# CuzImSlymi/Apertis-LLM

Hardware: AMD Instinct MI355X
Metric: train tokens/sec/node (seq=4096) (higher is better)
Workload: dtype bf16

## Files before the change

### apertis_llm_amd/csrc/moe_routing.hip

```cpp
#include "row_common.h"

namespace {

template <int EC>
__global__ void gate_topk_fwd_k(const float *__restrict__ logits, float *__restrict__ gates,
                                int32_t *__restrict__ idx, float *__restrict__ w, int64_t S, int E_rt,
                                int K) {
  const int64_t s = (int64_t)blockIdx.x * blockDim.x + threadIdx.x;
  if (s >= S) return;
  const int E = EC > 0 ? EC : E_rt;
  gate_topk_row<EC>(logits + s * E, gates + s * E, idx + s * K, w + s * K, E_rt, K);
}

template <int EC>
__global__ void gate_topk_bwd_k(const float *__restrict__ gates, const int32_t *__restrict__ idx,
                                const float *__restrict__ dw, const float *__restrict__ dgates,
                                float *__restrict__ dlogits, int64_t S, int E_rt, int K) {
  const int64_t s = (int64_t)blockIdx.x * blockDim.x + threadIdx.x;
  if (s >= S) return;
  constexpr int CAP = EC > 0 ? EC : MAXE;
  const int E = EC > 0 ? EC : E_rt;
  float g[CAP], dg[CAP];
#pragma unroll
  for (int i = 0; i < CAP; ++i)
    if (i < E) { g[i] = gates[s * E + i]; dg[i] = dgates ? dgates[s * E + i] : 0.f; }
  if (dw) {
    float psum = 0.f, dot = 0.f;
    for (int k = 0; k < K; ++k) {
      int e = idx[s * K + k];
      float pe = 0.f;
#pragma unroll
      for (int i = 0; i < CAP; ++i)
        if (i == e) pe = g[i];
      psum += pe;
      dot += dw[s * K + k] * pe;
    }
    const float den = psum + 1e-6f;
    const float corr = dot / (den * den);
    for (int k = 0; k < K; ++k) {
      int e = idx[s * K + k];
      float dp = dw[s * K + k] / den - corr;
#pragma unroll
      for (int i = 0; i < CAP; ++i)
        if (i == e) dg[i] += dp;
    }
  }
  float inner = 0.f;
#pragma unroll
  for (int i = 0; i < CAP; ++i)
    if (i < E) inner += dg[i] * g[i];
#pragma unroll
  for (int i = 0; i < CAP; ++i)
    if (i < E) dlogits[s * E + i] = g[i] * (dg[i] - inner);
}

constexpr int PLAN_HIST_BLOCKS = 512;
struct PlanWs {
  int32_t *total, *keep, *mode, *quota, *seg_start, *bpart;
  uint32_t *thr, *smask;
  int32_t *ghist;
  int32_t *done;
  int32_t *cnt_g, *cnt_t;
  int P, NCH;
};

PlanWs carve_ws(void *ws, int64_t S, int64_t E, int64_t K) {
  PlanWs w;
  w.P = (int)(E * K);
  w.NCH = (int)ceil_div64(S, 64);
  int32_t *p = (int32_t *)ws;
  w.total = p; p += w.P;
  w.keep = p; p += w.P;
  w.mode = p; p += w.P;
  w.quota = p; p += w.P;
  w.seg_start = p; p += w.P;
  w.thr = (uint32_t *)p; p += w.P;
  w.smask = (uint32_t *)p; p += w.P;
  w.ghist = p; p += (int64_t)w.P * 256;
  w.done = p; p += 4;
  w.cnt_g = p; p += (int64_t)w.P * w.NCH;
  w.cnt_t = p; p += (int64_t)w.P * w.NCH;
  w.bpart = p;
  return w;
}

__global__ void __launch_bounds__(256)
plan_hist_k(const int32_t *__restrict__ idx, int32_t *__restrict__ bpart, int64_t SK, int E, int K) {
  __shared__ int32_t h[MAXE * MAXK];
  const int P = E * K, lane = threadIdx.x & 63;
  for (int i = threadIdx.x; i < P; i += blockDim.x) h[i] = 0;
  __syncthreads();
  for (int64_t a0 = (int64_t)blockIdx.x * blockDim.x; a0 < SK; a0 += (int64_t)gridDim.x * blockDim.x) {
    const int64_t a = a0 + threadIdx.x;
    int slot = -1;
    if (a < SK) {
      const int e = idx[a];
      if (e >= 0 && e < E) slot = e * K + (int)(a % K);
    }
    unsigned long long todo = __ballot(slot >= 0);
    while (todo) {
      const int leader = __ffsll((long long)todo) - 1;
      const int s0 = __shfl(slot, leader);
      const unsigned long long m = __ballot(slot == s0);
      if (lane == leader) atomicAdd(&h[s0], __popcll(m));
      todo &= ~m;
    }
  }
  __syncthreads();
  for (int i = threadIdx.x; i < P; i += blockDim.x) bpart[(int64_t)blockIdx.x * P + i] = h[i];
}

__global__ void plan_capacity_k(PlanWs w, const uint8_t *__restrict__ active, int64_t capacity,
                                int32_t *__restrict__ offsets, int E, int K, int nhist) {
  __shared__ int32_t s_sum[256];
  {
    const int P = E * K;
    const int g = P < 256 ? 256 / P : 1;
    for (int p0 = 0; p0 < P; p0 += 256 / g) {
      const int p = p0 + (int)threadIdx.x / g, sub = (int)threadIdx.x % g;
      int t = 0;
      if (p < P && (int)threadIdx.x / g < 256 / g)
        for (int b = sub; b < nhist; b += g) t += w.bpart[(int64_t)b * P + p];
      s_sum[threadIdx.x] = t;
      __syncthreads();
      if (p < P && sub == 0 && (int)threadIdx.x / g < 256 / g) {
        int tt = 0;
        for (int q = 0; q < g; ++q) tt += s_sum[threadIdx.x + q];
        w.total[p] = tt;
      }
      __syncthreads();
    }
  }
  const int e = threadIdx.x;
  if (e < E) {
    int64_t load = 0;
    const bool on = active ? active[e] != 0 : true;
    for (int k = 0; k < K; ++k) {
      const int p = e * K + k;
      const int tot = w.total[p];
      int64_t keep = tot;
      if (!on) keep = 0;
      else if (capacity > 0) {
        int64_t rem = capacity - load;
        keep = rem <= 0 ? 0 : (tot < rem ? tot : rem);
      }
      w.keep[p] = (int)keep;
      w.mode[p] = keep == 0 ? 0 : (keep == tot ? 1 : 2);
      w.quota[p] = (int)keep;
      w.thr[p] = 0;
      w.smask[p] = 0;
      load += keep;
    }
  }
  __syncthreads();
  if (threadIdx.x == 0) {
    int run = 0;
    for (int ee = 0; ee < E; ++ee) {
      offsets[ee] = run;
      for (int k = 0; k < K; ++k) {
        w.seg_start[ee * K + k] = run;
        run += w.keep[ee * K + k];
      }
    }
    offsets[E] = run;
  }
}

__global__ void __launch_bounds__(1024)
plan_select_k(PlanWs w, const int32_t *__restrict__ idx, const float *__restrict__ wk, int64_t S, int K) {
  const int p = blockIdx.x;
  if (w.mode[p] != 2) return;
  const int e = p / K, k = p - e * K;
  __shared__ int32_t hist[256];
  __shared__ uint32_t s_prefix, s_mask;
  __shared__ int32_t s_need;
  if (threadIdx.x == 0) { s_prefix = 0; s_mask = 0; s_need = w.keep[p]; }
  for (int shift = 24; shift >= 0; shift -= 8) {
    for (int i = threadIdx.x; i < 256; i += blockDim.x) hist[i] = 0;
    __syncthreads();
    const uint32_t prefix = s_prefix, mask = s_mask;
    for (int64_t s0 = threadIdx.x; s0 < S; s0 += (int64_t)blockDim.x * 8) {
      int32_t ei[8];
      uint32_t bi[8];
#pragma unroll
      for (int u = 0; u < 8; ++u) {
        const int64_t s = s0 + (int64_t)u * blockDim.x;
        ei[u] = s < S ? idx[s * K + k] : -1;
        bi[u] = s < S ? __float_as_uint(wk[s * K + k]) : 0u;
      }
#pragma unroll
      for (int u = 0; u < 8; ++u)
        if (ei[u] == e && (bi[u] & mask) == prefix) atomicAdd(&hist[(bi[u] >> shift) & 255], 1);
    }
    __syncthreads();
    if (threadIdx.x == 0) {
      int need = s_need, cum = 0;
      for (int b = 255; b >= 0; --b) {
        if (cum + hist[b] >= need) {
          s_need = need - cum;
          s_prefix = prefix | ((uint32_t)b << shift);
          s_mask = mask | (255u << shift);
          break;
        }
        cum += hist[b];
      }
    }
    __syncthreads();
  }
  if (threadIdx.x == 0) { w.thr[p] = s_prefix; w.quota[p] = s_need; }
}

__device__ __forceinline__ void plan_sel_pick(const PlanWs &w, int p, int lane, int shift) {
  if (w.mode[p] != 2) return;
  int32_t *h = w.ghist + p * 256;
  int c[4];
#pragma unroll
  for (int j = 0; j < 4; ++j) c[j] = __hip_atomic_load(h + 255 - 4 * lane - j, __ATOMIC_RELAXED, __HIP_MEMORY_SCOPE_AGENT);
  const int mine = (c[0] + c[1]) + (c[2] + c[3]);
  int incl = mine;
#pragma unroll
  for (int off = 1; off < 64; off <<= 1) {
    const int v = __shfl_up(incl, off);
    if (lane >= off) incl += v;
  }
  const int need = w.quota[p];
  const int before = incl - mine;
  if (before < need && incl >= need) {
    int cum = before, b = 0;
#pragma unroll
    for (int j = 0; j < 4; ++j) {
      if (cum < need && cum + c[j] >= need) { b = 255 - 4 * lane - j; break; }
      cum += c[j];
    }
    w.quota[p] = need - cum;
    w.thr[p] = w.thr[p] | ((uint32_t)b << shift);
    w.smask[p] = w.smask[p] | (255u << shift);
  }
#pragma unroll
  for (int j = 0; j < 4; ++j) h[255 - 4 * lane - j] = 0;
}

__global__ void __launch_bounds__(256)
plan_sel_hist_k(PlanWs w, const int32_t *__restrict__ idx, const float *__restrict__ wk, int64_t S, int E, int K, int shift, int digit) {
  extern __shared__ int32_t lh[];
  __shared__ int32_t s_mode[32];
  __shared__ uint32_t s_mask[32], s_thr[32];
  const int P = w.P;
  for (int i = threadIdx.x; i < P * 256; i += 256) lh[i] = 0;
  if (threadIdx.x < P) { s_mode[threadIdx.x] = w.mode[threadIdx.x]; s_mask[threadIdx.x] = w.smask[threadIdx.x]; s_thr[threadIdx.x] = w.thr[threadIdx.x]; }
  __syncthreads();
  const int64_t SK = S * K;
  for (int64_t a0 = (int64_t)blockIdx.x * 256 + threadIdx.x; a0 < SK; a0 += (int64_t)gridDim.x * 256 * 4) {
    int32_t ei[4];
    uint32_t bi[4];
#pragma unroll
    for (int u = 0; u < 4; ++u) {
      const int64_t a = a0 + (int64_t)u * gridDim.x * 256;
      ei[u] = a < SK ? idx[a] : -1;
      bi[u] = a < SK ? __float_as_uint(wk[a]) : 0u;
    }
#pragma unroll
    for (int u = 0; u < 4; ++u) {
      const int64_t a = a0 + (int64_t)u * gridDim.x * 256;
      if (ei[u] >= 0 && ei[u] < E) {
        const int p = ei[u] * K + (int)(a % K);
        if (s_mode[p] == 2 && (bi[u] & s_mask[p]) == s_thr[p]) atomicAdd(&lh[p * 256 + ((bi[u] >> shift) & 255)], 1);
      }
    }
  }
  __syncthreads();
  for (int i = threadIdx.x; i < P * 256; i += 256)
    if (lh[i]) atomicAdd(&w.ghist[i], lh[i]);
  __threadfence();
  __syncthreads();
  __shared__ int s_last;
  if (threadIdx.x == 0) s_last = atomicAdd(&w.done[digit], 1) == (int)gridDim.x - 1;
  __syncthreads();
  if (!s_last) return;
  __threadfence();
  for (int p = threadIdx.x >> 6; p < P; p += 4) plan_sel_pick(w, p, threadIdx.x & 63, shift);
}

__device__ __forceinline__ void plan_flags(const PlanWs &w, const int32_t *idx, const float *wk, int64_t s,
                                           int64_t S, int k, int E, int K, int &e, bool &fg, bool &ft) {
  e = -1; fg = false; ft = false;
  if (s < S) {
    e = idx[s * K + k];
    if (e >= 0 && e < E) {
      const int p = e * K + k;
      const int m = w.mode[p];
      if (m == 1) fg = true;
      else if (m == 2) {
        uint32_t bits = __float_as_uint(wk[s * K + k]);
        uint32_t t = w.thr[p];
        fg = bits > t;
        ft = bits == t;
      }
    } else e = -1;
  }
}

__global__ void plan_count_k(PlanWs w, const int32_t *__restrict__ idx, const float *__restrict__ wk,
                             int64_t S, int E, int K) {
  const int lane = threadIdx.x & 63;
  const int64_t chunk = (int64_t)blockIdx.x * (blockDim.x >> 6) + (threadIdx.x >> 6);
  if (chunk >= w.NCH) return;
  const int64_t s = chunk * 64 + lane;
  for (int k = 0; k < K; ++k) {
    int e; bool fg, ft;
    plan_flags(w, idx, wk, s, S, k, E, K, e, fg, ft);
    for (int ee = 0; ee < E; ++ee) {
      unsigned long long bg = __ballot(e == ee && fg);
      unsigned long long bt = __ballot(e == ee && ft);
      if (lane == 0) {
        w.cnt_g[(int64_t)(ee * K + k) * w.NCH + chunk] = __popcll(bg);
        w.cnt_t[(int64_t)(ee * K + k) * w.NCH + chunk] = __popcll(bt);
      }
    }
  }
}

__global__ void __launch_bounds__(256) plan_scan_k(PlanWs w) {
  int32_t *arr = (blockIdx.x < (unsigned)w.P ? w.cnt_g + (int64_t)blockIdx.x * w.NCH
                                              : w.cnt_t + (int64_t)(blockIdx.x - w.P) * w.NCH);
  __shared__ int32_t part[256];
  const int per = (w.NCH + 255) / 256;
  const int b0 = threadIdx.x * per, b1 = min(b0 + per, w.NCH);
  int sum = 0;
  for (int i = b0; i < b1; ++i) sum += arr[i];
  part[threadIdx.x] = sum;
  __syncthreads();
  if (threadIdx.x == 0) {
    int run = 0;
    for (int i = 0; i < 256; ++i) { int t = part[i]; part[i] = run; run += t; }
  }
  __syncthreads();
  int run = part[threadIdx.x];
  for (int i = b0; i < b1; ++i) { int t = arr[i]; arr[i] = run; run += t; }
}

__global__ void plan_assign_k(PlanWs w, const int32_t *__restrict__ idx, const float *__restrict__ wk,
                              int32_t *__restrict__ row_token, int32_t *__restrict__ row_k,
                              int32_t *__restrict__ slot_of, int64_t S, int E, int K) {
  const int lane = threadIdx.x & 63;
  const int64_t chunk = (int64_t)blockIdx.x * (blockDim.x >> 6) + (threadIdx.x >> 6);
  if (chunk >= w.NCH) return;
  const int64_t s = chunk * 64 + lane;
  const unsigned long long lt = lane == 0 ? 0ull : (~0ull >> (64 - lane));
  for (int k = 0; k < K; ++k) {
    int e; bool fg, ft;
    plan_flags(w, idx, wk, s, S, k, E, K, e, fg, ft);
    int pre_g = 0, pre_t = 0;
    for (int ee = 0; ee < E; ++ee) {
      unsigned long long bg = __ballot(e == ee && fg);
      unsigned long long bt = __ballot(e == ee && ft);
      if (e == ee) { pre_g = __popcll(bg & lt); pre_t = __popcll(bt & lt); }
    }
    if (s < S) {
      int slot = -1;
      if (e >= 0 && (fg || ft)) {
        const int p = e * K + k;
        const int gb = w.cnt_g[(int64_t)p * w.NCH + chunk] + pre_g;
        const int tb = w.cnt_t[(int64_t)p * w.NCH + chunk] + pre_t;
        const int q = w.quota[p];
        if (fg || tb < q) {
          slot = w.seg_start[p] + gb + (tb < q ? tb : q);
          row_token[slot] = (int32_t)s;
          row_k[slot] = k;
        }
      }
      slot_of[s * K + k] = slot;
    }
  }
}

__global__ void __launch_bounds__(1024)
plan_small_k(const int32_t *__restrict__ idx, const float *__restrict__ wk, const uint8_t *__restrict__ active, int64_t capacity,
             int32_t *__restrict__ offsets, int32_t *__restrict__ row_token, int32_t *__restrict__ row_k,
             int32_t *__restrict__ slot_of, int S, int E, int K) {
  plan_small_body(idx, wk, active, capacity, offsets, row_token, row_k, slot_of, S, E, K, nullptr, nullptr);
}

__device__ __forceinline__ void gauss_pair(uint64_t seed, uint64_t pair, float &n0, float &n1) {
  const uint32_t h0 = drop_hash_pair(seed, 2 * pair), h1 = drop_hash_pair(seed ^ 0x9E3779B97F4A7C15ull, 2 * pair + 1);
  const float u1 = ((float)(h0 >> 8) + 1.0f) * (1.0f / 16777216.0f);
  const float u2 = (float)(h1 >> 8) * (1.0f / 16777216.0f);
  const float r = sqrtf(-2.0f * logf(u1));
  float sn, cs;
  sincospif(2.0f * u2, &sn, &cs);
  n0 = r * cs;
  n1 = r * sn;
}
__device__ __forceinline__ float softplus_gate(float x) { return x > 20.f ? x : log1pf(expf(x)); }
template <int CAP>
__device__ __forceinline__ void row_noise(uint64_t seed, int64_t s, int E, float (&nz)[CAP]) {
  const int64_t ppr = (E + 1) / 2;
#pragma unroll
  for (int i = 0; i < CAP; i += 2) {
    if (i < E) {
      float a, b;
      gauss_pair(seed, (uint64_t)(s * ppr + (i >> 1)), a, b);
      nz[i] = a;
      if (i + 1 < CAP) nz[i + 1] = b;
    }
  }
}

template <int EC>
__global__ void __launch_bounds__(256)
gate_topk_aux_fwd_k(const float *__restrict__ logits, const float *__restrict__ w_noise, float alpha, uint64_t seed,
                    float *__restrict__ gates, int32_t *__restrict__ idx,
                    float *__restrict__ w, float *__restrict__ lse, float *__restrict__ part, int64_t S, int E_rt, int K) {
  constexpr int CAP = EC > 0 ? EC : MAXE;
  const int E = EC > 0 ? EC : E_rt;
  const int64_t s = (int64_t)blockIdx.x * blockDim.x + threadIdx.x;
  const bool live = s < S;
  float v[CAP];
  float cnt[CAP];
  float l2 = 0.f;
#pragma unroll
  for (int i = 0; i < CAP; ++i) { v[i] = 0.f; cnt[i] = 0.f; }
  if (live) {
    const float *row = logits + s * E;
    float m = -INFINITY;
#pragma unroll
    for (int i = 0; i < CAP; ++i)
      if (i < E) v[i] = row[i];
    if (w_noise) {
      float nz[CAP];
      row_noise<CAP>(seed, s, E, nz);
#pragma unroll
      for (int i = 0; i < CAP; ++i)
        if (i < E) v[i] += nz[i] * (softplus_gate(w_noise[i]) * alpha);
    }
#pragma unroll
    for (int i = 0; i < CAP; ++i)
      if (i < E) m = fmaxf(m, v[i]);
    float sum = 0.f;
#pragma unroll
    for (int i = 0; i < CAP; ++i)
      if (i < E) { v[i] = expf(v[i] - m); sum += v[i]; }
    const float l = m + logf(sum);
    lse[s] = l;
    l2 = l * l;
#pragma unroll
    for (int i = 0; i < CAP; ++i)
      if (i < E) { v[i] = v[i] / sum; gates[s * E + i] = v[i]; }
    uint64_t chosen = 0;
    float p[MAXK];
    float psum = 0.f;
#pragma unroll
    for (int k = 0; k < MAXK; ++k) {
      if (k < K) {
        float best = -1.f;
        int bi = 0;
#pragma unroll
        for (int i = 0; i < CAP; ++i)
          if (i < E && !((chosen >> i) & 1) && v[i] > best) { best = v[i]; bi = i; }
        chosen |= 1ull << bi;
        idx[s * K + k] = bi;
        p[k] = best;
        psum += best;
      }
    }
    const float den = psum + 1e-6f;
#pragma unroll
    for (int k = 0; k < MAXK; ++k)
      if (k < K) w[s * K + k] = p[k] / den;
#pragma unroll
    for (int i = 0; i < CAP; ++i)
      if (i < E) cnt[i] = (float)((chosen >> i) & 1);
  }
  __shared__ float red[4][2 * MAXE + 1];
  const int lane = threadIdx.x & 63, wv = threadIdx.x >> 6;
#pragma unroll
  for (int i = 0; i < CAP; ++i) {
    if (i < E) {
      const float a = wave_sum(v[i]), b = wave_sum(cnt[i]);
      if (lane == 0) { red[wv][i] = a; red[wv][E + i] = b; }
    }
  }
  l2 = wave_sum(l2);
  if (lane == 0) red[wv][2 * E] = l2;
  __syncthreads();
  if (threadIdx.x < 2 * E + 1)
    part[(int64_t)blockIdx.x * (2 * E + 1) + threadIdx.x] =
        (red[0][threadIdx.x] + red[1][threadIdx.x]) + (red[2][threadIdx.x] + red[3][threadIdx.x]);
}

__global__ void __launch_bounds__(1024)
gate_aux_fold_k(const float *__restrict__ part, float *__restrict__ stats, int64_t nblk, int64_t S, int E, float lb_coef,
                float rz_coef) {
  __shared__ float tot[2 * MAXE + 1];
  const int lane = threadIdx.x & 63, wv = threadIdx.x >> 6;
  const int cols = 2 * E + 1;
  for (int cc = wv; cc < cols; cc += 16) {
    float a = 0.f;
    for (int64_t b = lane; b < nblk; b += 64) a += part[b * cols + cc];
    a = wave_sum(a);
    if (lane == 0) tot[cc] = a;
  }
  __syncthreads();
  if (threadIdx.x == 0) {
    float lb = 0.f;
    for (int e = 0; e < E; ++e) lb += (tot[E + e] / (float)S) * (tot[e] / (float)S);
    stats[0] = lb_coef * (float)E * lb;
    stats[1] = rz_coef * tot[2 * E] / (float)S;
  }
  if (threadIdx.x < E) stats[2 + threadIdx.x] = tot[E + threadIdx.x] / (float)S;
}

template <int EC>
__global__ void __launch_bounds__(256)
gate_topk_aux_bwd_k(const float *__restrict__ gates, const int32_t *__restrict__ idx,
                    const float *__restrict__ dw, const float *__restrict__ lse,
                    const float *__restrict__ stats, const float *__restrict__ dlb,
                    const float *__restrict__ drz, float lb_coef, float rz_coef,
                    float *__restrict__ dlogits, float *__restrict__ npart, uint64_t seed, int64_t S, int E_rt, int K) {
  const int64_t s = (int64_t)blockIdx.x * blockDim.x + threadIdx.x;
  constexpr int CAP = EC > 0 ? EC : MAXE;
  const int E = EC > 0 ? EC : E_rt;
  float dsc[CAP];
#pragma unroll
  for (int i = 0; i < CAP; ++i) dsc[i] = 0.f;
  if (s < S) {
  const float glb = dlb ? dlb[0] * lb_coef * (float)E / (float)S : 0.f;
  const float grz = drz ? drz[0] * rz_coef * 2.f * lse[s] / (float)S : 0.f;
  float g[CAP], dg[CAP];
#pragma unroll
  for (int i = 0; i < CAP; ++i)
    if (i < E) { g[i] = gates[s * E + i]; dg[i] = glb * stats[2 + i]; }
  if (dw) {
    float psum = 0.f, dot = 0.f;
    for (int k = 0; k < K; ++k) {
      int e = idx[s * K + k];
      float pe = 0.f;
#pragma unroll
      for (int i = 0; i < CAP; ++i)
        if (i == e) pe = g[i];
      psum += pe;
      dot += dw[s * K + k] * pe;
    }
    const float den = psum + 1e-6f;
    const float corr = dot / (den * den);
    for (int k = 0; k < K; ++k) {
      int e = idx[s * K + k];
      float dp = dw[s * K + k] / den - corr;
#pragma unroll
      for (int i = 0; i < CAP; ++i)
        if (i == e) dg[i] += dp;
    }
  }
  float inner = 0.f;
#pragma unroll
  for (int i = 0; i < CAP; ++i)
    if (i < E) inner += dg[i] * g[i];
  float nz[CAP];
  if (npart) row_noise<CAP>(seed, s, E, nz);
#pragma unroll
  for (int i = 0; i < CAP; ++i)
    if (i < E) {
      const float dl = g[i] * (dg[i] - inner) + grz * g[i];
      dlogits[s * E + i] = dl;
      if (npart) dsc[i] = dl * nz[i];
    }
  }
  if (npart) {
    __shared__ float red[4][MAXE];
    const int lane = threadIdx.x & 63, wv = threadIdx.x >> 6;
#pragma unroll
    for (int i = 0; i < CAP; ++i)
      if (i < E) {
        const float a = wave_sum(dsc[i]);
        if (lane == 0) red[wv][i] = a;
      }
    __syncthreads();
    if (threadIdx.x < E)
      npart[(int64_t)blockIdx.x * E + threadIdx.x] =
          (red[0][threadIdx.x] + red[1][threadIdx.x]) + (red[2][threadIdx.x] + red[3][threadIdx.x]);
  }
}

__global__ void __launch_bounds__(1024)
gate_noise_fold_k(const float *__restrict__ npart, const float *__restrict__ w_noise, float alpha, float *__restrict__ dw_noise,
                  int64_t nblk, int E) {
  const int lane = threadIdx.x & 63, wv = threadIdx.x >> 6;
  for (int e = wv; e < E; e += 16) {
    float a = 0.f;
    for (int64_t b = lane; b < nblk; b += 64) a += npart[b * E + e];
    a = wave_sum(a);
    if (lane == 0) {
      const float x = w_noise[e];
      dw_noise[e] = a * alpha * (x > 20.f ? 1.f : 1.f / (1.f + expf(-x)));
    }
  }
}

}

extern "C" int apertis_moe_gate_topk_fwd(const float *logits, float *gates, int32_t *idx, float *w,
                                         int64_t S, int64_t E, int64_t K, void *stream) {
  if (!logits || !gates || !idx || !w || S < 0) return APERTIS_ERR_ARG;
  if (E < 1 || E > MAXE || K < 1 || K > MAXK || K > E) return APERTIS_ERR_UNSUPPORTED;
  if (S == 0) return APERTIS_OK;
  hipStream_t st = (hipStream_t)stream;
  dim3 grid((unsigned)ceil_div64(S, 256)), block(256);
#define GO(EC) hipLaunchKernelGGL(gate_topk_fwd_k<EC>, grid, block, 0, st, logits, gates, idx, w, S, (int)E, (int)K)
  if (E == 4) GO(4); else if (E == 8) GO(8); else if (E == 16) GO(16); else GO(0);
#undef GO
  return apertis_check_launch();
}

extern "C" int apertis_moe_gate_topk_bwd(const float *gates, const int32_t *idx, const float *dw,
                                         const float *dgates, float *dlogits, int64_t S, int64_t E,
                                         int64_t K, void *stream) {
  if (!gates || !idx || !dlogits || S < 0) return APERTIS_ERR_ARG;
  if (E < 1 || E > MAXE || K < 1 || K > MAXK || K > E) return APERTIS_ERR_UNSUPPORTED;
  if (S == 0) return APERTIS_OK;
  hipStream_t st = (hipStream_t)stream;
  dim3 grid((unsigned)ceil_div64(S, 256)), block(256);
#define GO(EC) hipLaunchKernelGGL(gate_topk_bwd_k<EC>, grid, block, 0, st, gates, idx, dw, dgates, dlogits, S, (int)E, (int)K)
  if (E == 4) GO(4); else if (E == 8) GO(8); else if (E == 16) GO(16); else GO(0);
#undef GO
  return apertis_check_launch();
}

extern "C" int64_t apertis_moe_plan_workspace_bytes(int64_t S, int64_t E, int64_t K) {
  int64_t P = E * K, NCH = ceil_div64(S > 0 ? S : 1, 64);
  return (7 * P + 256 * P + 4 + 2 * P * NCH + PLAN_HIST_BLOCKS * P) * 4 + 64;
}

extern "C" int apertis_moe_plan(const int32_t *idx, const float *w, const uint8_t *active,
                                int64_t capacity, int32_t *expert_offsets, int32_t *row_token,
                                int32_t *row_k, int32_t *slot_of, void *ws, int64_t S, int64_t E,
                                int64_t K, void *stream) {
  if (!idx || !w || !expert_offsets || !row_token || !row_k || !slot_of || !ws || S < 0) return APERTIS_ERR_ARG;
  if (E < 1 || E > MAXE || K < 1 || K > MAXK) return APERTIS_ERR_UNSUPPORTED;
  if (S * K > 0x7fffffffLL) return APERTIS_ERR_UNSUPPORTED;
  hipStream_t st = (hipStream_t)stream;
  if (S > 0 && S <= 64 && E * K <= 16) {
    hipLaunchKernelGGL(plan_small_k, dim3(1), dim3(64 * (unsigned)(E * K)), 0, st, idx, w, active, capacity, expert_offsets,
                       row_token, row_k, slot_of, (int)S, (int)E, (int)K);
    return apertis_check_launch();
  }
  PlanWs pw = carve_ws(ws, S > 0 ? S : 1, E, K);
  int nhist = 0;
  if (S > 0) {
    nhist = (int)std::min<int64_t>(ceil_div64(S * K, 1024), PLAN_HIST_BLOCKS);
    hipLaunchKernelGGL(plan_hist_k, dim3((unsigned)nhist), dim3(256), 0, st, idx, pw.bpart, S * K, (int)E, (int)K);
  }
  hipLaunchKernelGGL(plan_capacity_k, dim3(1), dim3(256), 0, st, pw, active, capacity, expert_offsets, (int)E, (int)K, nhist);
  if (S > 0) {
    if (capacity > 0) {
      if (pw.P <= 32) {
        hipMemsetAsync(pw.ghist, 0, sizeof(int32_t) * (pw.P * 256 + 4), st);
        const unsigned nbh = (unsigned)std::min<int64_t>(ceil_div64(S * K, 1024), 512);
        for (int shift = 24; shift >= 0; shift -= 8)
          hipLaunchKernelGGL(plan_sel_hist_k, dim3(nbh), dim3(256), (size_t)pw.P * 256 * sizeof(int32_t), st, pw, idx, w, S,
                             (int)E, (int)K, shift, 3 - shift / 8);
      } else {
        hipLaunchKernelGGL(plan_select_k, dim3(pw.P), dim3(1024), 0, st, pw, idx, w, S, (int)K);
      }
    }
    dim3 cgrid((unsigned)ceil_div64(pw.NCH, 4)), cblock(256);
    hipLaunchKernelGGL(plan_count_k, cgrid, cblock, 0, st, pw, idx, w, S, (int)E, (int)K);
    hipLaunchKernelGGL(plan_scan_k, dim3(2 * pw.P), dim3(256), 0, st, pw);
    hipLaunchKernelGGL(plan_assign_k, cgrid, cblock, 0, st, pw, idx, w, row_token, row_k, slot_of, S, (int)E, (int)K);
  }
  return apertis_check_launch();
}

extern "C" int64_t apertis_moe_gate_aux_blocks(int64_t S) { return ceil_div64(S > 0 ? S : 1, 256); }

extern "C" int apertis_moe_gate_topk_noisy_aux_fwd(const float *logits, const float *w_noise, float alpha, uint64_t seed,
                                                   float *gates, int32_t *idx, float *w, float *lse, float *part, float *stats,
                                                   int64_t S, int64_t E, int64_t K, float lb_coef, float rz_coef, void *stream) {
  if (!logits || !gates || !idx || !w || !lse || !part || !stats || S <= 0) return APERTIS_ERR_ARG;
  if (E < 1 || E > MAXE || K < 1 || K > MAXK || K > E) return APERTIS_ERR_UNSUPPORTED;
  hipStream_t st = (hipStream_t)stream;
  const int64_t nblk = apertis_moe_gate_aux_blocks(S);
  dim3 grid((unsigned)nblk), block(256);
#define GO(EC) hipLaunchKernelGGL(gate_topk_aux_fwd_k<EC>, grid, block, 0, st, logits, w_noise, alpha, seed, gates, idx, w, lse, part, S, (int)E, (int)K)
  if (E == 4) GO(4); else if (E == 8) GO(8); else if (E == 16) GO(16); else GO(0);
#undef GO
  hipLaunchKernelGGL(gate_aux_fold_k, dim3(1), dim3(1024), 0, st, part, stats, nblk, S, (int)E, lb_coef, rz_coef);
  return apertis_check_launch();
}

extern "C" int apertis_moe_gate_topk_aux_fwd(const float *logits, float *gates, int32_t *idx, float *w, float *lse,
                                             float *part, float *stats, int64_t S, int64_t E, int64_t K, float lb_coef,
                                             float rz_coef, void *stream) {
  return apertis_moe_gate_topk_noisy_aux_fwd(logits, nullptr, 0.f, 0, gates, idx, w, lse, part, stats, S, E, K, lb_coef, rz_coef,
                                             stream);
}

extern "C" int apertis_moe_gate_topk_noisy_aux_bwd(const float *gates, const int32_t *idx, const float *dw, const float *lse,
                                                   const float *stats, const float *dlb, const float *drz, float lb_coef,
                                                   float rz_coef, const float *w_noise, float alpha, uint64_t seed,
                                                   float *dlogits, float *npart, float *dw_noise, int64_t S, int64_t E,
                                                   int64_t K, void *stream) {
  if (!gates || !idx || !lse || !stats || !dlogits || S < 0 || (w_noise && (!npart || !dw_noise))) return APERTIS_ERR_ARG;
  if (!w_noise) npart = nullptr;
  if (E < 1 || E > MAXE || K < 1 || K > MAXK || K > E) return APERTIS_ERR_UNSUPPORTED;
  if (S == 0) return APERTIS_OK;
  hipStream_t st = (hipStream_t)stream;
  dim3 grid((unsigned)ceil_div64(S, 256)), block(256);
#define GO(EC) hipLaunchKernelGGL(gate_topk_aux_bwd_k<EC>, grid, block, 0, st, gates, idx, dw, lse, stats, dlb, drz, lb_coef, rz_coef, dlogits, npart, seed, S, (int)E, (int)K)
  if (E == 4) GO(4); else if (E == 8) GO(8); else if (E == 16) GO(16); else GO(0);
#undef GO
  if (npart) hipLaunchKernelGGL(gate_noise_fold_k, dim3(1), dim3(1024), 0, st, npart, w_noise, alpha, dw_noise, (int64_t)grid.x, (int)E);
  return apertis_check_launch();
}

extern "C" int apertis_moe_gate_topk_aux_bwd(const float *gates, const int32_t *idx, const float *dw, const float *lse,
                                             const float *stats, const float *dlb, const float *drz, float lb_coef,
                                             float rz_coef, float *dlogits, int64_t S, int64_t E, int64_t K, void *stream) {
  return apertis_moe_gate_topk_noisy_aux_bwd(gates, idx, dw, lse, stats, dlb, drz, lb_coef, rz_coef, nullptr, 0.f, 0, dlogits,
                                             nullptr, nullptr, S, E, K, stream);
}
```

Measured before the change: 403,900.

## Restructure MoE routing plan into staged per-slot bucketing with fused selection

Replaces the multi-kernel routing plan (histogram, capacity, iterative radix-select passes, count, scan, assign) with a two- or three-kernel pipeline. A staging kernel buckets each (token, k) entry by expert slot into a compacted workspace. A per-slot kernel then scans the chunk counts, computes capacity, runs the radix threshold selection over only that slot's entries (held in LDS when they fit), and writes the assignments. This cuts kernel launches and repeated full passes over idx/weights. In exchange it uses more workspace (2*S*K extra) and puts more serial work into one block per slot.

```diff
diff --git a/apertis_llm_amd/csrc/moe_routing.hip b/apertis_llm_amd/csrc/moe_routing.hip
--- a/apertis_llm_amd/csrc/moe_routing.hip
+++ b/apertis_llm_amd/csrc/moe_routing.hip
@@ -54,324 +54,361 @@
     if (i < E) dlogits[s * E + i] = g[i] * (dg[i] - inner);
 }
 
-constexpr int PLAN_HIST_BLOCKS = 512;
+constexpr int PLAN_CHUNK = 1024;
+constexpr int PLAN_LOCAL_P = 32;
+constexpr int PLAN_LDS_ELEMS = (160 * 1024 - 4 * 1024) / 4;
+
 struct PlanWs {
-  int32_t *total, *keep, *mode, *quota, *seg_start, *bpart;
-  uint32_t *thr, *smask;
-  int32_t *ghist;
-  int32_t *done;
-  int32_t *cnt_g, *cnt_t;
+  int32_t *total, *keep, *seg_start;
+  int32_t *cnt, *pre;
+  int32_t *base;
+  int32_t *cg, *ct;
+  int32_t *st_tok;
+  uint32_t *st_bits;
   int P, NCH;
 };
 
 PlanWs carve_ws(void *ws, int64_t S, int64_t E, int64_t K) {
   PlanWs w;
   w.P = (int)(E * K);
-  w.NCH = (int)ceil_div64(S, 64);
+  w.NCH = (int)ceil_div64(S * K, PLAN_CHUNK);
+  const int64_t PN = (int64_t)w.P * w.NCH;
   int32_t *p = (int32_t *)ws;
   w.total = p; p += w.P;
   w.keep = p; p += w.P;
-  w.mode = p; p += w.P;
-  w.quota = p; p += w.P;
   w.seg_start = p; p += w.P;
-  w.thr = (uint32_t *)p; p += w.P;
-  w.smask = (uint32_t *)p; p += w.P;
-  w.ghist = p; p += (int64_t)w.P * 256;
-  w.done = p; p += 4;
-  w.cnt_g = p; p += (int64_t)w.P * w.NCH;
-  w.cnt_t = p; p += (int64_t)w.P * w.NCH;
-  w.bpart = p;
+  w.cnt = p; p += PN;
+  w.pre = p; p += PN;
+  w.base = p; p += PN + w.P;
+  w.cg = p; p += PN;
+  w.ct = p; p += PN;
+  w.st_tok = p; p += S * K;
+  w.st_bits = (uint32_t *)p;
   return w;
 }
 
+template <int NW>
+__device__ __forceinline__ int block_excl_scan(int v, int32_t *s_w, int &total) {
+  const int lane = threadIdx.x & 63, wv = threadIdx.x >> 6;
+  int incl = v;
+#pragma unroll
+  for (int off = 1; off < 64; off <<= 1) {
+    const int t = __shfl_up(incl, off);
+    if (lane >= off) incl += t;
+  }
+  if (lane == 63) s_w[wv] = incl;
+  __syncthreads();
+  int before = 0, all = 0;
+#pragma unroll
+  for (int i = 0; i < NW; ++i) {
+    const int t = s_w[i];
+    if (i < wv) before += t;
+    all += t;
+  }
+  __syncthreads();
+  total = all;
+  return before + incl - v;
+}
+
 __global__ void __launch_bounds__(256)
-plan_hist_k(const int32_t *__restrict__ idx, int32_t *__restrict__ bpart, int64_t SK, int E, int K) {
-  __shared__ int32_t h[MAXE * MAXK];
-  const int P = E * K, lane = threadIdx.x & 63;
-  for (int i = threadIdx.x; i < P; i += blockDim.x) h[i] = 0;
-  __syncthreads();
-  for (int64_t a0 = (int64_t)blockIdx.x * blockDim.x; a0 < SK; a0 += (int64_t)gridDim.x * blockDim.x) {
-    const int64_t a = a0 + threadIdx.x;
-    int slot = -1;
-    if (a < SK) {
-      const int e = idx[a];
-      if (e >= 0 && e < E) slot = e * K + (int)(a % K);
-    }
-    unsigned long long todo = __ballot(slot >= 0);
+plan_stage_k(PlanWs w, const int32_t *__restrict__ idx, const float *__restrict__ wk, int32_t *__restrict__ slot_of,
+             int64_t SK, int E, int K) {
+  extern __shared__ int32_t s_cnt[];
+  __shared__ int32_t s_w[4];
+  const int P = E * K, lane = threadIdx.x & 63, wv = threadIdx.x >> 6;
+  int32_t *s_pre = s_cnt + 16 * P;
+  for (int i = threadIdx.x; i < 16 * P; i += 256) s_cnt[i] = 0;
+  const int64_t a0 = (int64_t)blockIdx.x * PLAN_CHUNK;
+  int32_t ei[4];
+  uint32_t bi[4];
+#pragma unroll
+  for (int j = 0; j < 4; ++j) {
+    const int64_t a = a0 + j * 256 + threadIdx.x;
+    ei[j] = a < SK ? idx[a] : -1;
+    bi[j] = a < SK ? __float_as_uint(wk[a]) : 0u;
+  }
+  __syncthreads();
+  const unsigned long long lt = lane == 0 ? 0ull : (~0ull >> (64 - lane));
+  int slot[4], rank[4];
+#pragma unroll
+  for (int j = 0; j < 4; ++j) {
+    const int64_t a = a0 + j * 256 + threadIdx.x;
+    slot[j] = -1;
+    rank[j] = 0;
+    if (ei[j] >= 0 && ei[j] < E) slot[j] = ei[j] * K + (int)((uint32_t)a % (uint32_t)K);
+    else if (a < SK) slot_of[a] = -1;
+    unsigned long long todo = __ballot(slot[j] >= 0);
     while (todo) {
       const int leader = __ffsll((long long)todo) - 1;
-      const int s0 = __shfl(slot, leader);
-      const unsigned long long m = __ballot(slot == s0);
-      if (lane == leader) atomicAdd(&h[s0], __popcll(m));
+      const int s0 = __shfl(slot[j], leader);
+      const unsigned long long m = __ballot(slot[j] == s0);
+      if (slot[j] == s0) rank[j] = __popcll(m & lt);
+      if (lane == leader) s_cnt[(j * 4 + wv) * P + s0] = __popcll(m);
       todo &= ~m;
     }
   }
   __syncthreads();
-  for (int i = threadIdx.x; i < P; i += blockDim.x) bpart[(int64_t)blockIdx.x * P + i] = h[i];
-}
-
-__global__ void plan_capacity_k(PlanWs w, const uint8_t *__restrict__ active, int64_t capacity,
-                                int32_t *__restrict__ offsets, int E, int K, int nhist) {
-  __shared__ int32_t s_sum[256];
-  {
-    const int P = E * K;
-    const int g = P < 256 ? 256 / P : 1;
-    for (int p0 = 0; p0 < P; p0 += 256 / g) {
-      const int p = p0 + (int)threadIdx.x / g, sub = (int)threadIdx.x % g;
-      int t = 0;
-      if (p < P && (int)threadIdx.x / g < 256 / g)
-        for (int b = sub; b < nhist; b += g) t += w.bpart[(int64_t)b * P + p];
-      s_sum[threadIdx.x] = t;
-      __syncthreads();
-      if (p < P && sub == 0 && (int)threadIdx.x / g < 256 / g) {
-        int tt = 0;
-        for (int q = 0; q < g; ++q) tt += s_sum[threadIdx.x + q];
-        w.total[p] = tt;
-      }
-      __syncthreads();
-    }
-  }
+  const int per = (P + 255) / 256;
+  int mine = 0;
+  for (int q = 0; q < per; ++q) {
+    const int p = threadIdx.x * per + q;
+    if (p < P) {
+      int run = 0;
+#pragma unroll
+      for (int g = 0; g < 16; ++g) { const int t = s_cnt[g * P + p]; s_cnt[g * P + p] = run; run += t; }
+      s_pre[p] = run;
+      mine += run;
+    }
+  }
+  int all;
+  int run = block_excl_scan<4>(mine, s_w, all);
+  for (int q = 0; q < per; ++q) {
+    const int p = threadIdx.x * per + q;
+    if (p < P) {
+      const int t = s_pre[p];
+      s_pre[p] = run;
+      w.cnt[(int64_t)p * w.NCH + blockIdx.x] = t;
+      w.pre[(int64_t)p * w.NCH + blockIdx.x] = run;
+      run += t;
+    }
+  }
+  __syncthreads();
+#pragma unroll
+  for (int j = 0; j < 4; ++j) {
+    if (slot[j] >= 0) {
+      const int64_t a = a0 + j * 256 + threadIdx.x;
+      const int64_t d = a0 + s_pre[slot[j]] + s_cnt[(j * 4 + wv) * P + slot[j]] + rank[j];
+      w.st_tok[d] = (int32_t)((uint32_t)a / (uint32_t)K);
+      w.st_bits[d] = bi[j];
+    }
+  }
+}
+
+__device__ __forceinline__ void plan_capacity_body(const int32_t *tot, int32_t *keep, int32_t *seg, const uint8_t *__restrict__ active,
+                                                   int64_t capacity, int32_t *__restrict__ offsets, int E, int K) {
   const int e = threadIdx.x;
   if (e < E) {
     int64_t load = 0;
     const bool on = active ? active[e] != 0 : true;
     for (int k = 0; k < K; ++k) {
-      const int p = e * K + k;
-      const int tot = w.total[p];
-      int64_t keep = tot;
-      if (!on) keep = 0;
+      const int t = tot[e * K + k];
+      int64_t kp = t;
+      if (!on) kp = 0;
       else if (capacity > 0) {
-        int64_t rem = capacity - load;
-        keep = rem <= 0 ? 0 : (tot < rem ? tot : rem);
+        const int64_t rem = capacity - load;
+        kp = rem <= 0 ? 0 : (t < rem ? t : rem);
       }
-      w.keep[p] = (int)keep;
-      w.mode[p] = keep == 0 ? 0 : (keep == tot ? 1 : 2);
-      w.quota[p] = (int)keep;
-      w.thr[p] = 0;
-      w.smask[p] = 0;
-      load += keep;
+      keep[e * K + k] = (int)kp;
+      load += kp;
     }
   }
   __syncthreads();
   if (threadIdx.x == 0) {
     int run = 0;
     for (int ee = 0; ee < E; ++ee) {
-      offsets[ee] = run;
-      for (int k = 0; k < K; ++k) {
-        w.seg_start[ee * K + k] = run;
-        run += w.keep[ee * K + k];
-      }
-    }
-    offsets[E] = run;
+      if (offsets) offsets[ee] = run;
+      for (int k = 0; k < K; ++k) { seg[ee * K + k] = run; run += keep[ee * K + k]; }
+    }
+    if (offsets) offsets[E] = run;
+  }
+  __syncthreads();
+}
+
+__device__ __forceinline__ void plan_totals(const PlanWs &w, int32_t *tot) {
+  const int lane = threadIdx.x & 63;
+  for (int q = threadIdx.x >> 6; q < w.P; q += 16) {
+    const int32_t *row = w.cnt + (int64_t)q * w.NCH;
+    int t = 0;
+    for (int c = lane; c < w.NCH; c += 64) t += row[c];
+#pragma unroll
+    for (int off = 32; off > 0; off >>= 1) t += __shfl_xor(t, off);
+    if (lane == 0) tot[q] = t;
   }
 }
 
 __global__ void __launch_bounds__(1024)
-plan_select_k(PlanWs w, const int32_t *__restrict__ idx, const float *__restrict__ wk, int64_t S, int K) {
-  const int p = blockIdx.x;
-  if (w.mode[p] != 2) return;
-  const int e = p / K, k = p - e * K;
-  __shared__ int32_t hist[256];
+plan_capacity_k(PlanWs w, const uint8_t *__restrict__ active, int64_t capacity, int32_t *__restrict__ offsets, int E, int K) {
+  plan_totals(w, w.total);
+  __syncthreads();
+  plan_capacity_body(w.total, w.keep, w.seg_start, active, capacity, offsets, E, K);
+}
+
+template <typename F>
+__device__ __forceinline__ void plan_runs(const int32_t *base, const int32_t *pre, const int32_t *xs, const int32_t *ys, int NCH, F f) {
+  const int lane = threadIdx.x & 63, wv = threadIdx.x >> 6;
+  for (int cb = 0; cb < NCH; cb += 1024) {
+    const int cm = cb + lane * 16 + wv;
+    int mb = 0, ml = 0, ms = 0, mx = 0, my = 0;
+    if (cm < NCH) {
+      mb = base[cm];
+      ml = base[cm + 1] - mb;
+      ms = pre[cm];
+      if (xs) mx = xs[cm];
+      if (ys) my = ys[cm];
+    }
+    for (int l = 0; l < 64; ++l) {
+      const int c = cb + l * 16 + wv;
+      if (c >= NCH) break;
+      f(c, __shfl(mb, l), __shfl(ml, l), (int64_t)c * PLAN_CHUNK + __shfl(ms, l), __shfl(mx, l), __shfl(my, l));
+    }
+  }
+}
+
+__device__ __forceinline__ void plan_digit_count(int32_t *hist, bool ok, uint32_t bits, uint32_t mask, uint32_t prefix, int shift) {
+  const int lane = threadIdx.x & 63;
+  int d = ok && (bits & mask) == prefix ? (int)((bits >> shift) & 255u) : -1;
+  unsigned long long todo = __ballot(d >= 0);
+  for (int it = 0; it < 3 && todo; ++it) {
+    const int leader = __ffsll((long long)todo) - 1;
+    const int d0 = __shfl(d, leader);
+    const unsigned long long m = __ballot(d == d0);
+    if (lane == leader) atomicAdd(&hist[d0], __popcll(m));
+    if (d == d0) d = -1;
+    todo &= ~m;
+  }
+  if (d >= 0) atomicAdd(&hist[d], 1);
+}
+
+__global__ void __launch_bounds__(1024)
+plan_slot_k(PlanWs w, const uint8_t *__restrict__ active, int64_t capacity, int32_t *__restrict__ offsets,
+            int32_t *__restrict__ row_token, int32_t *__restrict__ row_k, int32_t *__restrict__ slot_of, int E, int K, int lds_elems) {
+  extern __shared__ uint32_t s_bits[];
+  __shared__ int32_t s_wsum[16], s_hist[256], s_tot[PLAN_LOCAL_P], s_keep[PLAN_LOCAL_P], s_seg[PLAN_LOCAL_P];
   __shared__ uint32_t s_prefix, s_mask;
   __shared__ int32_t s_need;
-  if (threadIdx.x == 0) { s_prefix = 0; s_mask = 0; s_need = w.keep[p]; }
+  const int p = blockIdx.x, k = p % K, NCH = w.NCH, lane = threadIdx.x & 63;
+  const int32_t *cnt = w.cnt + (int64_t)p * NCH, *pre = w.pre + (int64_t)p * NCH;
+  int32_t *base = w.base + (int64_t)p * (NCH + 1), *cg = w.cg + (int64_t)p * NCH, *ct = w.ct + (int64_t)p * NCH;
+  int n = 0;
+  for (int c0 = 0; c0 < NCH; c0 += 1024) {
+    const int c = c0 + threadIdx.x;
+    int all;
+    const int ex = block_excl_scan<16>(c < NCH ? cnt[c] : 0, s_wsum, all);
+    if (c < NCH) base[c] = n + ex;
+    n += all;
+  }
+  if (threadIdx.x == 0) base[NCH] = n;
+  int keep, seg;
+  if (w.P <= PLAN_LOCAL_P) {
+    plan_totals(w, s_tot);
+    __syncthreads();
+    plan_capacity_body(s_tot, s_keep, s_seg, active, capacity, p == 0 ? offsets : nullptr, E, K);
+    keep = s_keep[p];
+    seg = s_seg[p];
+  } else {
+    keep = w.keep[p];
+    seg = w.seg_start[p];
+    __syncthreads();
+  }
+  if (keep == 0 || keep == n) {
+    plan_runs(base, pre, nullptr, nullptr, NCH, [&](int, int b, int len, int64_t at, int, int) {
+      for (int i = lane; i < len; i += 64) {
+        const int tok = w.st_tok[at + i];
+        const int row = keep ? seg + b + i : -1;
+        if (row >= 0) { row_token[row] = tok; row_k[row] = k; }
+        slot_of[(int64_t)tok * K + k] = row;
+      }
+    });
+    return;
+  }
+  const bool in_lds = n <= lds_elems;
+  if (in_lds)
+    plan_runs(base, pre, nullptr, nullptr, NCH, [&](int, int b, int len, int64_t at, int, int) {
+      for (int i = lane; i < len; i += 64) s_bits[b + i] = w.st_bits[at + i];
+    });
+  if (threadIdx.x == 0) { s_prefix = 0; s_mask = 0; s_need = keep; }
   for (int shift = 24; shift >= 0; shift -= 8) {
-    for (int i = threadIdx.x; i < 256; i += blockDim.x) hist[i] = 0;
+    if (threadIdx.x < 256) s_hist[threadIdx.x] = 0;
     __syncthreads();
     const uint32_t prefix = s_prefix, mask = s_mask;
-    for (int64_t s0 = threadIdx.x; s0 < S; s0 += (int64_t)blockDim.x * 8) {
-      int32_t ei[8];
-      uint32_t bi[8];
-#pragma unroll
-      for (int u = 0; u < 8; ++u) {
-        const int64_t s = s0 + (int64_t)u * blockDim.x;
-        ei[u] = s < S ? idx[s * K + k] : -1;
-        bi[u] = s < S ? __float_as_uint(wk[s * K + k]) : 0u;
+    if (in_lds) {
+      for (int j0 = 0; j0 < n; j0 += 1024) {
+        const int j = j0 + threadIdx.x;
+        plan_digit_count(s_hist, j < n, j < n ? s_bits[j] : 0u, mask, prefix, shift);
       }
-#pragma unroll
-      for (int u = 0; u < 8; ++u)
-        if (ei[u] == e && (bi[u] & mask) == prefix) atomicAdd(&hist[(bi[u] >> shift) & 255], 1);
+    } else {
+      plan_runs(base, pre, nullptr, nullptr, NCH, [&](int, int, int len, int64_t at, int, int) {
+        for (int i0 = 0; i0 < len; i0 += 64) {
+          const int i = i0 + lane;
+          plan_digit_count(s_hist, i < len, i < len ? w.st_bits[at + i] : 0u, mask, prefix, shift);
+        }
+      });
     }
     __syncthreads();
-    if (threadIdx.x == 0) {
-      int need = s_need, cum = 0;
-      for (int b = 255; b >= 0; --b) {
-        if (cum + hist[b] >= need) {
-          s_need = need - cum;
-          s_prefix = prefix | ((uint32_t)b << shift);
-          s_mask = mask | (255u << shift);
-          break;
+    if (threadIdx.x < 64) {
+      int c[4];
+#pragma unroll
+      for (int j = 0; j < 4; ++j) c[j] = s_hist[255 - 4 * lane - j];
+      const int mine = (c[0] + c[1]) + (c[2] + c[3]);
+      int incl = mine;
+#pragma unroll
+      for (int off = 1; off < 64; off <<= 1) {
+        const int v = __shfl_up(incl, off);
+        if (lane >= off) incl += v;
+      }
+      const int need = s_need, before = incl - mine;
+      if (before < need && incl >= need) {
+        int cum = before, bsel = 0;
+#pragma unroll
+        for (int j = 0; j < 4; ++j) {
+          if (cum + c[j] >= need) { bsel = 255 - 4 * lane - j; break; }
+          cum += c[j];
         }
-        cum += hist[b];
+        s_need = need - cum;
+        s_prefix = prefix | ((uint32_t)bsel << shift);
+        s_mask = mask | (255u << shift);
       }
     }
     __syncthreads();
   }
-  if (threadIdx.x == 0) { w.thr[p] = s_prefix; w.quota[p] = s_need; }
-}
-
-__device__ __forceinline__ void plan_sel_pick(const PlanWs &w, int p, int lane, int shift) {
-  if (w.mode[p] != 2) return;
-  int32_t *h = w.ghist + p * 256;
-  int c[4];
-#pragma unroll
-  for (int j = 0; j < 4; ++j) c[j] = __hip_atomic_load(h + 255 - 4 * lane - j, __ATOMIC_RELAXED, __HIP_MEMORY_SCOPE_AGENT);
-  const int mine = (c[0] + c[1]) + (c[2] + c[3]);
-  int incl = mine;
-#pragma unroll
-  for (int off = 1; off < 64; off <<= 1) {
-    const int v = __shfl_up(incl, off);
-    if (lane >= off) incl += v;
-  }
-  const int need = w.quota[p];
-  const int before = incl - mine;
-  if (before < need && incl >= need) {
-    int cum = before, b = 0;
-#pragma unroll
-    for (int j = 0; j < 4; ++j) {
-      if (cum < need && cum + c[j] >= need) { b = 255 - 4 * lane - j; break; }
-      cum += c[j];
-    }
-    w.quota[p] = need - cum;
-    w.thr[p] = w.thr[p] | ((uint32_t)b << shift);
-    w.smask[p] = w.smask[p] | (255u << shift);
-  }
-#pragma unroll
-  for (int j = 0; j < 4; ++j) h[255 - 4 * lane - j] = 0;
-}
-
-__global__ void __launch_bounds__(256)
-plan_sel_hist_k(PlanWs w, const int32_t *__restrict__ idx, const float *__restrict__ wk, int64_t S, int E, int K, int shift, int digit) {
-  extern __shared__ int32_t lh[];
-  __shared__ int32_t s_mode[32];
-  __shared__ uint32_t s_mask[32], s_thr[32];
-  const int P = w.P;
-  for (int i = threadIdx.x; i < P * 256; i += 256) lh[i] = 0;
-  if (threadIdx.x < P) { s_mode[threadIdx.x] = w.mode[threadIdx.x]; s_mask[threadIdx.x] = w.smask[threadIdx.x]; s_thr[threadIdx.x] = w.thr[threadIdx.x]; }
-  __syncthreads();
-  const int64_t SK = S * K;
-  for (int64_t a0 = (int64_t)blockIdx.x * 256 + threadIdx.x; a0 < SK; a0 += (int64_t)gridDim.x * 256 * 4) {
-    int32_t ei[4];
-    uint32_t bi[4];
-#pragma unroll
-    for (int u = 0; u < 4; ++u) {
-      const int64_t a = a0 + (int64_t)u * gridDim.x * 256;
-      ei[u] = a < SK ? idx[a] : -1;
-      bi[u] = a < SK ? __float_as_uint(wk[a]) : 0u;
-    }
-#pragma unroll
-    for (int u = 0; u < 4; ++u) {
-      const int64_t a = a0 + (int64_t)u * gridDim.x * 256;
-      if (ei[u] >= 0 && ei[u] < E) {
-        const int p = ei[u] * K + (int)(a % K);
-        if (s_mode[p] == 2 && (bi[u] & s_mask[p]) == s_thr[p]) atomicAdd(&lh[p * 256 + ((bi[u] >> shift) & 255)], 1);
+  const uint32_t thr = s_prefix;
+  const int quota = s_need;
+  const unsigned long long lt = lane == 0 ? 0ull : (~0ull >> (64 - lane));
+  plan_runs(base, pre, nullptr, nullptr, NCH, [&](int c, int b, int len, int64_t at, int, int) {
+    int ng = 0, nt = 0;
+    for (int i0 = 0; i0 < len; i0 += 64) {
+      const int i = i0 + lane;
+      const uint32_t bits = i < len ? (in_lds ? s_bits[b + i] : w.st_bits[at + i]) : 0u;
+      ng += __popcll(__ballot(i < len && bits > thr));
+      nt += __popcll(__ballot(i < len && bits == thr));
+    }
+    if (lane == 0) { cg[c] = ng; ct[c] = nt; }
+  });
+  __syncthreads();
+  {
+    int rg = 0, rt = 0;
+    for (int c0 = 0; c0 < NCH; c0 += 1024) {
+      const int c = c0 + threadIdx.x;
+      int ag, at;
+      const int eg = block_excl_scan<16>(c < NCH ? cg[c] : 0, s_wsum, ag);
+      const int et = block_excl_scan<16>(c < NCH ? ct[c] : 0, s_wsum, at);
+      if (c < NCH) { cg[c] = rg + eg; ct[c] = rt + et; }
+      rg += ag;
+      rt += at;
+    }
+  }
+  __syncthreads();
+  plan_runs(base, pre, cg, ct, NCH, [&](int, int b, int len, int64_t at, int gb, int tb) {
+    for (int i0 = 0; i0 < len; i0 += 64) {
+      const int i = i0 + lane;
+      const uint32_t bits = i < len ? (in_lds ? s_bits[b + i] : w.st_bits[at + i]) : 0u;
+      const bool fg = i < len && bits > thr, ft = i < len && bits == thr;
+      const unsigned long long bg = __ballot(fg), bt = __ballot(ft);
+      if (i < len) {
+        const int tok = w.st_tok[at + i];
+        const int ti = tb + __popcll(bt & lt);
+        int row = -1;
+        if (fg || (ft && ti < quota)) {
+          row = seg + gb + __popcll(bg & lt) + (ti < quota ? ti : quota);
+          row_token[row] = tok;
+          row_k[row] = k;
+        }
+        slot_of[(int64_t)tok * K + k] = row;
       }
-    }
-  }
-  __syncthreads();
-  for (int i = threadIdx.x; i < P * 256; i += 256)
-    if (lh[i]) atomicAdd(&w.ghist[i], lh[i]);
-  __threadfence();
-  __syncthreads();
-  __shared__ int s_last;
-  if (threadIdx.x == 0) s_last = atomicAdd(&w.done[digit], 1) == (int)gridDim.x - 1;
-  __syncthreads();
-  if (!s_last) return;
-  __threadfence();
-  for (int p = threadIdx.x >> 6; p < P; p += 4) plan_sel_pick(w, p, threadIdx.x & 63, shift);
-}
-
-__device__ __forceinline__ void plan_flags(const PlanWs &w, const int32_t *idx, const float *wk, int64_t s,
-                                           int64_t S, int k, int E, int K, int &e, bool &fg, bool &ft) {
-  e = -1; fg = false; ft = false;
-  if (s < S) {
-    e = idx[s * K + k];
-    if (e >= 0 && e < E) {
-      const int p = e * K + k;
-      const int m = w.mode[p];
-      if (m == 1) fg = true;
-      else if (m == 2) {
-        uint32_t bits = __float_as_uint(wk[s * K + k]);
-        uint32_t t = w.thr[p];
-        fg = bits > t;
-        ft = bits == t;
-      }
-    } else e = -1;
-  }
-}
-
-__global__ void plan_count_k(PlanWs w, const int32_t *__restrict__ idx, const float *__restrict__ wk,
-                             int64_t S, int E, int K) {
-  const int lane = threadIdx.x & 63;
-  const int64_t chunk = (int64_t)blockIdx.x * (blockDim.x >> 6) + (threadIdx.x >> 6);
-  if (chunk >= w.NCH) return;
-  const int64_t s = chunk * 64 + lane;
-  for (int k = 0; k < K; ++k) {
-    int e; bool fg, ft;
-    plan_flags(w, idx, wk, s, S, k, E, K, e, fg, ft);
-    for (int ee = 0; ee < E; ++ee) {
-      unsigned long long bg = __ballot(e == ee && fg);
-      unsigned long long bt = __ballot(e == ee && ft);
-      if (lane == 0) {
-        w.cnt_g[(int64_t)(ee * K + k) * w.NCH + chunk] = __popcll(bg);
-        w.cnt_t[(int64_t)(ee * K + k) * w.NCH + chunk] = __popcll(bt);
-      }
-    }
-  }
-}
-
-__global__ void __launch_bounds__(256) plan_scan_k(PlanWs w) {
-  int32_t *arr = (blockIdx.x < (unsigned)w.P ? w.cnt_g + (int64_t)blockIdx.x * w.NCH
-                                              : w.cnt_t + (int64_t)(blockIdx.x - w.P) * w.NCH);
-  __shared__ int32_t part[256];
-  const int per = (w.NCH + 255) / 256;
-  const int b0 = threadIdx.x * per, b1 = min(b0 + per, w.NCH);
-  int sum = 0;
-  for (int i = b0; i < b1; ++i) sum += arr[i];
-  part[threadIdx.x] = sum;
-  __syncthreads();
-  if (threadIdx.x == 0) {
-    int run = 0;
-    for (int i = 0; i < 256; ++i) { int t = part[i]; part[i] = run; run += t; }
-  }
-  __syncthreads();
-  int run = part[threadIdx.x];
-  for (int i = b0; i < b1; ++i) { int t = arr[i]; arr[i] = run; run += t; }
-}
-
-__global__ void plan_assign_k(PlanWs w, const int32_t *__restrict__ idx, const float *__restrict__ wk,
-                              int32_t *__restrict__ row_token, int32_t *__restrict__ row_k,
-                              int32_t *__restrict__ slot_of, int64_t S, int E, int K) {
-  const int lane = threadIdx.x & 63;
-  const int64_t chunk = (int64_t)blockIdx.x * (blockDim.x >> 6) + (threadIdx.x >> 6);
-  if (chunk >= w.NCH) return;
-  const int64_t s = chunk * 64 + lane;
-  const unsigned long long lt = lane == 0 ? 0ull : (~0ull >> (64 - lane));
-  for (int k = 0; k < K; ++k) {
-    int e; bool fg, ft;
-    plan_flags(w, idx, wk, s, S, k, E, K, e, fg, ft);
-    int pre_g = 0, pre_t = 0;
-    for (int ee = 0; ee < E; ++ee) {
-      unsigned long long bg = __ballot(e == ee && fg);
-      unsigned long long bt = __ballot(e == ee && ft);
-      if (e == ee) { pre_g = __popcll(bg & lt); pre_t = __popcll(bt & lt); }
-    }
-    if (s < S) {
-      int slot = -1;
-      if (e >= 0 && (fg || ft)) {
-        const int p = e * K + k;
-        const int gb = w.cnt_g[(int64_t)p * w.NCH + chunk] + pre_g;
-        const int tb = w.cnt_t[(int64_t)p * w.NCH + chunk] + pre_t;
-        const int q = w.quota[p];
-        if (fg || tb < q) {
-          slot = w.seg_start[p] + gb + (tb < q ? tb : q);
-          row_token[slot] = (int32_t)s;
-          row_k[slot] = k;
-        }
-      }
-      slot_of[s * K + k] = slot;
-    }
-  }
+      gb += __popcll(bg);
+      tb += __popcll(bt);
+    }
+  });
 }
 
 __global__ void __launch_bounds__(1024)
@@ -626,8 +663,8 @@
 }
 
 extern "C" int64_t apertis_moe_plan_workspace_bytes(int64_t S, int64_t E, int64_t K) {
-  int64_t P = E * K, NCH = ceil_div64(S > 0 ? S : 1, 64);
-  return (7 * P + 256 * P + 4 + 2 * P * NCH + PLAN_HIST_BLOCKS * P) * 4 + 64;
+  const int64_t SK = (S > 0 ? S : 0) * K, P = E * K, NCH = ceil_div64(SK, PLAN_CHUNK);
+  return (3 * P + 5 * P * NCH + P + 2 * SK) * 4 + 64;
 }
 
 extern "C" int apertis_moe_plan(const int32_t *idx, const float *w, const uint8_t *active,
@@ -643,30 +680,15 @@
                        row_token, row_k, slot_of, (int)S, (int)E, (int)K);
     return apertis_check_launch();
   }
-  PlanWs pw = carve_ws(ws, S > 0 ? S : 1, E, K);
-  int nhist = 0;
-  if (S > 0) {
-    nhist = (int)std::min<int64_t>(ceil_div64(S * K, 1024), PLAN_HIST_BLOCKS);
-    hipLaunchKernelGGL(plan_hist_k, dim3((unsigned)nhist), dim3(256), 0, st, idx, pw.bpart, S * K, (int)E, (int)K);
-  }
-  hipLaunchKernelGGL(plan_capacity_k, dim3(1), dim3(256), 0, st, pw, active, capacity, expert_offsets, (int)E, (int)K, nhist);
-  if (S > 0) {
-    if (capacity > 0) {
-      if (pw.P <= 32) {
-        hipMemsetAsync(pw.ghist, 0, sizeof(int32_t) * (pw.P * 256 + 4), st);
-        const unsigned nbh = (unsigned)std::min<int64_t>(ceil_div64(S * K, 1024), 512);
-        for (int shift = 24; shift >= 0; shift -= 8)
-          hipLaunchKernelGGL(plan_sel_hist_k, dim3(nbh), dim3(256), (size_t)pw.P * 256 * sizeof(int32_t), st, pw, idx, w, S,
-                             (int)E, (int)K, shift, 3 - shift / 8);
-      } else {
-        hipLaunchKernelGGL(plan_select_k, dim3(pw.P), dim3(1024), 0, st, pw, idx, w, S, (int)K);
-      }
-    }
-    dim3 cgrid((unsigned)ceil_div64(pw.NCH, 4)), cblock(256);
-    hipLaunchKernelGGL(plan_count_k, cgrid, cblock, 0, st, pw, idx, w, S, (int)E, (int)K);
-    hipLaunchKernelGGL(plan_scan_k, dim3(2 * pw.P), dim3(256), 0, st, pw);
-    hipLaunchKernelGGL(plan_assign_k, cgrid, cblock, 0, st, pw, idx, w, row_token, row_k, slot_of, S, (int)E, (int)K);
-  }
+  PlanWs pw = carve_ws(ws, S, E, K);
+  if (S > 0)
+    launch_lds(plan_stage_k, dim3((unsigned)pw.NCH), dim3(256), (size_t)17 * pw.P * sizeof(int32_t), st, pw, idx, w, slot_of, S * K,
+               (int)E, (int)K);
+  if (pw.P > PLAN_LOCAL_P)
+    hipLaunchKernelGGL(plan_capacity_k, dim3(1), dim3(1024), 0, st, pw, active, capacity, expert_offsets, (int)E, (int)K);
+  const int lds_elems = capacity > 0 ? (int)std::min<int64_t>(S, PLAN_LDS_ELEMS) : 0;
+  launch_lds(plan_slot_k, dim3((unsigned)pw.P), dim3(1024), (size_t)lds_elems * sizeof(uint32_t), st, pw, active, capacity,
+             expert_offsets, row_token, row_k, slot_of, (int)E, (int)K, lds_elems);
   return apertis_check_launch();
 }
 
```

After: 403,000. About the same (-0.2%).
